# google-research/snap

Hardware: AMD Instinct MI355X
Metric: localization_scenes_per_sec (higher is better)
Workload: dtype f32 (tensors, accumulation, every non-GEMM op); conv / dense products on the bf16 matrix cores: operands split into 2 bf16 parts, 3 part products per MAC, ~2^-17 per product; 1 GPU; C2: 8 scenes/GPU, 4 StreetView views @512px + aerial, 128x128x60 voxel BEV @0.2m, ResNet-50 encoders, 10001 pose hypotheses; scenes_per_gpu=8, batches_in_flight=2, global_batch=8, parallelism=scene-sharded x1, no data-path collective, mode=inference forward (BEVLocalizer.apply, train=False)

## Files before the change

include/snap_hip.h:

```cpp
#ifndef SNAP_HIP_H_
#define SNAP_HIP_H_

#include <stddef.h>
#include <stdint.h>

#ifdef __cplusplus
extern "C" {
#endif

typedef enum SnapStatus {
  SNAP_OK = 0,
  SNAP_ERR_BAD_SHAPE = -1,
  SNAP_ERR_UNSUPPORTED = -2,
  SNAP_ERR_NULL = -3,
  SNAP_ERR_LAUNCH = -4,
  SNAP_ERR_WORKSPACE = -5
} SnapStatus;

int snap_abi_version(void);
const char* snap_status_string(int status);
const char* snap_build_arch(void);

enum { SNAP_PRO_NONE = 0, SNAP_PRO_AFFINE = 1, SNAP_PRO_GN_RELU = 2,
       SNAP_PRO_RELU_GN = 3, SNAP_PRO_RELU = 4 };
// ... 369 lines not shown

size_t snap_pose_score_workspace_bytes(int32_t B, int32_t Nq, int32_t P,
                                       int32_t X, int32_t Y);
int snap_pose_score_f32(const float* sim, const float* poses, const float* q_xy,
                        const uint8_t* valid_q, const uint8_t* map_valid,
                        int32_t B, int32_t Nq, int32_t X, int32_t Y, int32_t P,
                        float cell_size, int32_t mask_oob, float* scores,
                        void* workspace, size_t workspace_bytes, void* stream);

int snap_refine_lattice_f32(const float* init, const float* offs_r,
                            const float* offs_p, int32_t B, int32_t nr,
                            int32_t np_, float* out, void* stream);

int snap_argmax_rows_f32(const float* scores, int32_t B, int32_t P, int32_t start,
                         int32_t* idx, void* stream);

int snap_rotate_templates_f32(const float* feat, const uint8_t* valid,
                              const float* tfm, int32_t H, int32_t W, int32_t D,
                              int32_t R, float cell_size, float* templates,
                              uint8_t* tvalid, float* tw, float* cw,
                              float* tcount, void* stream);

int snap_stack_templates_f32(const float* tw, float* tws, int32_t H, int32_t W, int32_t D,
                             int32_t R, int32_t S, void* stream);
int snap_stack_templates_rhwd_f32(const float* templates, float* tws, int32_t H, int32_t W,
                                  int32_t D, int32_t R, int32_t S, void* stream);
int snap_pack_stacked_templates_split_bf16(const float* templates, int32_t H, int32_t W, int32_t D,
                                           int32_t R, int32_t S, void* out, size_t out_bytes,
                                           void* stream);
int snap_pad_map_f32(const float* map, const uint8_t* mvalid, int32_t H, int32_t W,
// ... 241 lines not shown
```

snap_amd/_lib.py:

```python
import ctypes
import os

_HERE = os.path.dirname(os.path.abspath(__file__))
LIB_PATH = os.environ.get('SNAP_HIP_LIB') or os.path.join(_HERE, 'lib', 'libsnap_hip.so')

c_int = ctypes.c_int32
c_i64 = ctypes.c_int64
c_u64 = ctypes.c_uint64
c_float = ctypes.c_float
c_size = ctypes.c_size_t
ptr = ctypes.c_void_p


class SnapConvDesc(ctypes.Structure):
  _fields_ = [
      ('N', c_int), ('H', c_int), ('W', c_int), ('Cin', c_int),
      ('Cin_stride', c_int),
      ('KH', c_int), ('KW', c_int), ('stride', c_int), ('pad_t', c_int),
      ('pad_l', c_int),
      ('Ho', c_int), ('Wo', c_int), ('Cout', c_int), ('Cout_stride', c_int),
      ('prologue', c_int), ('epilogue', c_int),
      ('in_scale', c_float), ('in_shift', c_float), ('tile_hint', c_int),
  ]

# ... 9 lines not shown
      ('bk_hint', c_int), ('tune_flags', c_int), ('gn_partial_rows', c_int), ('w_half', c_int), ('x_half', c_int), ('y_half', ptr),
      ('gnb_x', ptr), ('gnb_mu', ptr), ('gnb_rstd', ptr), ('gnb_gamma', ptr), ('gnb_beta', ptr), ('gnb_mode', c_int),
  ]


class SnapLiftDesc(ctypes.Structure):
  _fields_ = [
      ('B', c_int), ('V', c_int), ('h', c_int), ('w', c_int), ('C', c_int),
      ('feature_dim', c_int), ('num_bins', c_int), ('N', c_int), ('K', c_int),
      ('fisheye', c_int), ('out_stride', c_int),
      ('depth_min', c_float), ('depth_max', c_float),
      ('max_view_distance', c_float),
      ('weighted', c_int), ('use_variance', c_int), ('add_minmax', c_int),
      ('grid_y', c_int), ('grid_z', c_int), ('valid_rows_only', c_int), ('out_split', c_int),
      ('class_rows', c_int), ('tune_flags', c_int),
  ]


SIGNATURES = {
    'snap_abi_version': (c_int, []),
    'snap_status_string': (ctypes.c_char_p, [c_int]),
    'snap_build_arch': (ctypes.c_char_p, []),
    'snap_conv2d_nhwc_f32': (
        c_int,
        [ctypes.POINTER(SnapConvDesc), ptr, ptr, ptr, ptr, ptr, ptr, ptr, ptr,
         ptr, ptr, ptr],
    ),
    'snap_conv2d_nhwc_ex_f32': (
        c_int,
        [ctypes.POINTER(SnapConvDesc), ptr, ptr, ptr, ptr, ptr, ptr, ptr, ptr,
# ... 174 lines not shown
    'snap_poses_from_corr_f32': (
        c_int, [ptr, ptr, c_int, c_int, c_int, c_int, c_float, ptr, ptr]
    ),
    'snap_pose_score_window_workspace_bytes': (c_size, [c_int, c_int, c_int, c_int, c_int]),
    'snap_pose_score_window_supported': (c_int, [c_int, c_int, c_int]),
    'snap_pose_score_window_f32': (c_int, [ptr, ptr, ptr, c_int, ptr, ptr, c_int, c_int, c_int, c_int, c_int,
                                           c_float, ptr, ptr, c_size, ptr]),
    'snap_pose_score_workspace_bytes': (c_size, [c_int, c_int, c_int, c_int, c_int]),
    'snap_pose_score_f32': (
        c_int,
        [ptr, ptr, ptr, ptr, ptr, c_int, c_int, c_int, c_int, c_int, c_float,
         c_int, ptr, ptr, c_size, ptr],
    ),
    'snap_refine_lattice_f32': (c_int, [ptr, ptr, ptr, c_int, c_int, c_int, ptr, ptr]),
    'snap_argmax_rows_f32': (c_int, [ptr, c_int, c_int, c_int, ptr, ptr]),
    'snap_rotate_templates_f32': (
        c_int,
        [ptr, ptr, ptr, c_int, c_int, c_int, c_int, c_float, ptr, ptr, ptr, ptr,
         ptr, ptr],
    ),
    'snap_pad_map_f32': (c_int, [ptr, ptr, c_int, c_int, c_int, ptr, ptr, ptr]),
    'snap_template_finalize_f32': (
        c_int, [ptr, ptr, ptr, c_int, c_int, c_int, c_int, c_float, c_int, ptr, ptr]
    ),
    'snap_vote_peaks_workspace_bytes': (c_size, [c_int] * 6),
    'snap_vote_peaks_f32': (c_int, [ptr, c_int, c_int, c_int, c_int, c_int, c_int, ptr, ptr, ptr, ptr, c_size, ptr]),
    'snap_vote_posterior_workspace_bytes': (c_size, [c_int] * 3),
    'snap_vote_posterior_f32': (c_int, [ptr, c_int, c_int, c_int, c_float, ptr, ptr, ptr, ptr, ptr, ptr, c_size, ptr]),
    'snap_vote_fuse_workspace_bytes': (c_size, [c_int] * 4),
    'snap_vote_fuse_f32': (c_int, [ptr, ptr, ptr, c_int, c_int, c_int, c_int, ptr, ptr, ptr, c_size, ptr]),
# ... 96 lines not shown
    'snap_pose_score_bwd_f32': (
        c_int,
        [ptr, ptr, ptr, ptr, ptr, c_int, c_int, c_int, c_int, c_int, c_float, c_int, ptr, ptr,
         c_size, ptr],
    ),
    'snap_pose_score_bwd_ex_f32': (
        c_int,
        [ptr, ptr, ptr, ptr, ptr, c_int, c_int, c_int, c_int, c_int, c_float, c_int, c_int, ptr, ptr,
         c_size, ptr],
    ),
    'snap_sim_bwd_prepare_f32': (
        c_int, [ptr, ptr, c_int, c_i64, c_int, ptr, ptr, c_int, ptr]
    ),
}

ABI_VERSION = 27

_lib = None


def load():
  global _lib
  if _lib is not None:
    return _lib
  if not os.path.exists(LIB_PATH):
    raise RuntimeError(
        f'{LIB_PATH} not found: the HIP extension is not built. '
        'Run `make -C snap_amd/csrc` (needs hipcc); there is no CPU fallback.'
    )
  lib = ctypes.CDLL(LIB_PATH)
  for name, (restype, argtypes) in SIGNATURES.items():
# ... 16 lines not shown
```

snap_amd/csrc/abi.hip:

```cpp
#include "common.h"

extern "C" int snap_abi_version(void) { return 27; }

extern "C" const char* snap_build_arch(void) { return "gfx950"; }

extern "C" const char* snap_status_string(int status) {
  switch (status) {
    case SNAP_OK: return "ok";
    case SNAP_ERR_BAD_SHAPE: return "bad or inconsistent shape";
    case SNAP_ERR_UNSUPPORTED: return "unsupported option";
    case SNAP_ERR_NULL: return "required pointer is NULL";
    case SNAP_ERR_LAUNCH: return "HIP launch error";
    case SNAP_ERR_WORKSPACE: return "workspace too small";
    default: return "unknown status";
  }
}
```

snap_amd/csrc/pose.hip:

```cpp
#include <stdlib.h>

#include "common.h"
#include "philox.h"

namespace {

constexpr int SIM_CH = 64;
constexpr int SIM_TQ = 64;

template <int DM, int MODE>
__global__ __launch_bounds__(256) void sim_kernel(
    const float* __restrict__ fq, const float* __restrict__ fm, int Nq, int XY, float scale,
    int clip, const float* __restrict__ num_valid, float* __restrict__ sim,
    float* __restrict__ stats, const float* __restrict__ rowstats, float* __restrict__ prob,
    const float* __restrict__ row_weight) {
  __shared__ float q_s[SIM_TQ * DM];
  const int b = blockIdx.z;
  const int n0 = blockIdx.y * SIM_TQ;
  const int cell = blockIdx.x * 256 + threadIdx.x;
  const int lane = threadIdx.x & 63;
  const int chunk = blockIdx.x * 4 + (threadIdx.x >> 6);
  const int NC = (XY + SIM_CH - 1) / SIM_CH;
  const bool cvalid = cell < XY;
  for (int i = threadIdx.x; i < SIM_TQ * DM; i += 256) {
// ... 1305 lines not shown
  const float c = cosf(th0), s = sinf(th0);
  const float ox = offs_p[ix], oy = offs_p[iy];
  out[i * 3 + 0] = th0 + offs_r[ir];
  out[i * 3 + 1] = tx0 + (c * ox - s * oy);
  out[i * 3 + 2] = ty0 + (s * ox + c * oy);
}

__device__ __forceinline__ bool argmax_takes(float ov, int oi, float mv, int mi) {
  const bool on = ov != ov, mn = mv != mv;
  if (on != mn) return on;
  return (on || ov == mv) ? oi < mi : ov > mv;
}

template <int NT>
__global__ __launch_bounds__(NT) void argmax_rows_kernel(const float* __restrict__ scores, int P,
                                                         int start, int32_t* __restrict__ idx) {
  __shared__ float bv[NT];
  __shared__ int bi[NT];
  const int b = blockIdx.x;
  const float* row = scores + (int64_t)b * P;
  float best = -INFINITY;
  int besti = 0x7fffffff;
  for (int p = start + threadIdx.x; p < P; p += NT) {
    const float v = row[p];
    if (argmax_takes(v, p, best, besti)) { best = v; besti = p; }
  }
  bv[threadIdx.x] = best;
  bi[threadIdx.x] = besti;
  __syncthreads();
  for (int o = NT / 2; o > 0; o >>= 1) {
    if (threadIdx.x < o) {
      const float ov = bv[threadIdx.x + o];
      const int oi = bi[threadIdx.x + o];
      const float mv = bv[threadIdx.x];
      const int mi = bi[threadIdx.x];
      if (argmax_takes(ov, oi, mv, mi)) {
        bv[threadIdx.x] = ov;
        bi[threadIdx.x] = oi;
      }
    }
    __syncthreads();
  }
  if (threadIdx.x == 0) idx[b] = bi[0] - start;
}

template <int MODE>
int launch_sim(int Dm, dim3 grid, hipStream_t s, const float* fq, const float* fm, int Nq, int XY,
               float scale, int clip, const float* nv, float* sim, float* stats,
               const float* rowstats, float* prob, const float* row_weight) {
  switch (Dm) {
    case 8: hipLaunchKernelGGL((sim_kernel<8, MODE>), grid, dim3(256), 0, s, fq, fm, Nq, XY, scale, clip, nv, sim, stats, rowstats, prob, row_weight); break;
    case 16: hipLaunchKernelGGL((sim_kernel<16, MODE>), grid, dim3(256), 0, s, fq, fm, Nq, XY, scale, clip, nv, sim, stats, rowstats, prob, row_weight); break;
    case 32: hipLaunchKernelGGL((sim_kernel<32, MODE>), grid, dim3(256), 0, s, fq, fm, Nq, XY, scale, clip, nv, sim, stats, rowstats, prob, row_weight); break;
    case 64: hipLaunchKernelGGL((sim_kernel<64, MODE>), grid, dim3(256), 0, s, fq, fm, Nq, XY, scale, clip, nv, sim, stats, rowstats, prob, row_weight); break;
    default: return SNAP_ERR_UNSUPPORTED;
  }
  SNAP_CHECK_LAUNCH();
  return SNAP_OK;
// ... 334 lines not shown
  if (!init || !offs_r || !offs_p || !out) return SNAP_ERR_NULL;
  if (B <= 0 || nr <= 0 || np_ <= 0) return SNAP_ERR_BAD_SHAPE;
  const int64_t total = (int64_t)B * nr * np_ * np_;
  hipLaunchKernelGGL(refine_lattice_kernel, dim3((unsigned)snap_cdiv(total, 256)), dim3(256), 0,
                     static_cast<hipStream_t>(stream), init, offs_r, offs_p, B, nr, np_, out);
  SNAP_CHECK_LAUNCH();
  return SNAP_OK;
}

extern "C" int snap_argmax_rows_f32(const float* scores, int32_t B, int32_t P, int32_t start,
                                    int32_t* idx, void* stream) {
  if (!scores || !idx) return SNAP_ERR_NULL;
  if (B <= 0 || P <= 0 || start < 0 || start >= P) return SNAP_ERR_BAD_SHAPE;
  if (P - start > 4096)
    hipLaunchKernelGGL(argmax_rows_kernel<1024>, dim3(B), dim3(1024), 0, static_cast<hipStream_t>(stream),
                       scores, P, start, idx);
  else
    hipLaunchKernelGGL(argmax_rows_kernel<256>, dim3(B), dim3(256), 0, static_cast<hipStream_t>(stream),
                       scores, P, start, idx);
  SNAP_CHECK_LAUNCH();
  return SNAP_OK;
}
```

snap_amd/models/bev_localizer.py:

```python
import math

import numpy as np
import torch

from snap_amd import autograd as ag
from snap_amd import ops
from snap_amd.configs import defaults as default_configs
from snap_amd.models import base
from snap_amd.models import bev_mapper
from snap_amd.models import pose_estimation
from snap_amd.models import types
from snap_amd.utils import geometry
from snap_amd.utils import grids


def build_query_frustum_grid(cell_size, depth, filter_points_in_fov=False, hfov_deg=None):
  width = 3 * depth // 2
  grid = grids.Grid2D.from_extent_meters((width, depth), cell_size)
  grid_p_view = torch.tensor([width / 2, 0.0], dtype=torch.float32)
  qgrid_xy_p = grid.index_to_xyz(grid.grid_index().to(torch.float32))
  q_xy_p = qgrid_xy_p - grid_p_view
  if filter_points_in_fov:
    angle = torch.atan2(q_xy_p[..., 0], q_xy_p[..., 1])
    keep = torch.abs(angle) < math.radians(hfov_deg / 2)
# ... 83 lines not shown
        features=[f[: B * V].reshape(B, V, *f.shape[1:]) for f in pyr.features],
        strides=pyr.strides,
    )
    data_query['image_feature_pyr'] = types.FeatureImagePyramid(
        features=[f[B * V:].reshape(B, Vq, *f.shape[1:]) for f in pyr.features],
        strides=pyr.strides,
    )

  def _prefetch_scale(self, params):
    if self.config.add_temperature:
      ops.prefetch_exp(params.get('temperature'))

  def similarity(self, params, f_p_q, plane_map, valid_points, want_prob=False, conf_p=None):
    cfg = self.config
    temperature = params['temperature'] if cfg.add_temperature else None
    num_valid = valid_points.sum(-1).clamp(min=1).to(torch.float32)
    fq, fm = f_p_q.contiguous(), plane_map.features.contiguous()
    clip = bool(cfg.clip_negative_scores)
    weights = row_cdf = None
    train_w = conf_p is not None and base.needs_grad(fq, fm, temperature, conf_p)
    if conf_p is not None:
      if train_w:
        weights, row_cdf = ag.masked_softmax_rows(conf_p, valid_points)
      else:
        weights, row_cdf = ops.masked_softmax_rows(conf_p.contiguous(), valid_points.contiguous())
    if train_w:
      sim, stats, prob, scale = ag.sim_softmax_weighted(fq, fm, temperature, weights, clip, num_valid,
                                                        want_prob)
      weights, row_cdf = weights.detach(), row_cdf.detach()
    elif base.needs_grad(fq, fm, temperature):
      sim, stats, prob, scale = ag.sim_softmax(fq, fm, temperature, clip, num_valid, want_prob)
    else:
      scale = 1.0 if temperature is None else ops.host_exp(temperature)
      sim, stats, prob, _ = ops.sim_softmax(fq, fm, scale, clip, num_valid, want_prob=want_prob,
                                            row_weight=weights)
    if weights is not None:
      row_unscale = torch.where(weights > 0, 1.0 / weights.clamp(min=1e-38), torch.zeros_like(weights))
    else:
      row_unscale = num_valid[:, None].expand(-1, fq.shape[1]).contiguous()
    matching = dict(fq=fq.detach(), fm=fm.detach(), chunk_stats=stats, scale=scale, clip=clip,
                    row_cdf=row_cdf, sim=sim.detach(), row_unscale=row_unscale.contiguous())
    return sim, prob, matching

  def __call__(self, params, data, train=False, debug=False, rng=None,
               pose_samples=None):
    cfg = self.config
    ctx = base.ForwardContext()
    dev = data['query']['images'].device
    batch_size = len(data['query']['images'])
    q_xy_p = base.device_const('q_xy_p', dev, lambda: self.q_xy_p, owner=self)[None].expand(
        batch_size, -1, -1, -1)

    pred = {}
    data_map, data_query = dict(data['map']), {**data['query'], 'xy_bev': q_xy_p}
    self._prefetch_scale(params)
    self.bev_mapper.start_aerial(params['bev_mapper'], data_map, train, ctx)
    try:
      self._encode_views_jointly(params, data_map, data_query, train, ctx)
      pred['map'] = self.bev_mapper(params['bev_mapper'], data_map, train, debug, ctx=ctx, rng=rng)
    finally:
      pending = data_map.pop('_aerial_async', None)
      if pending is not None:
        torch.cuda.current_stream().wait_event(pending[1])
    mapper_q = self.bev_mapper_query or self.bev_mapper
    params_q = params['bev_mapper_query'] if self.bev_mapper_query is not None else params['bev_mapper']
    pred['query'] = mapper_q(
        params_q, data_query, train, debug, is_query=True, ctx=ctx, rng=rng,
    )

    plane_map = pred['map']['bev_matching']
    plane_q = pred['query']['bev_matching']
    q_xy_p = q_xy_p.squeeze(2).contiguous()
    valid_points = plane_q.valid.reshape(batch_size, -1)
    f_p_q = plane_q.features.reshape(batch_size, -1, plane_q.features.shape[-1])

    conf_p = None
    if cfg.add_confidence_query:
      conf_p = pred['query']['bev_confidence'].reshape(batch_size, -1)
    sim_points, prob_points, matching = self.similarity(
        params, f_p_q, plane_map, valid_points, want_prob=debug, conf_p=conf_p
    )
    if debug:
      pred['sim_points'] = sim_points
      pred['prob_points'] = prob_points

    if pose_samples is None:
      if cfg.num_pose_samples is None:
        raise ValueError('config.num_pose_samples must be set')
      m_t_q, corr = pose_estimation.sample_transforms_ransac_batched(
          rng, matching, q_xy_p, cfg.num_pose_samples,
          cfg.num_pose_sampling_retries, self.grid_map,
      )
      if debug:
        pred['correspondences'] = corr
    else:
      m_t_q = pose_samples
    m_t_q_gt = data.get('T_query2map')
    if m_t_q_gt is not None:
      m_t_q_gt = geometry.Transform2D.from_Transform3D(m_t_q_gt)
      m_t_q = geometry.Transform2D.cat([m_t_q_gt[:, None], m_t_q], 1)
    pred['map_t_query_samples'] = m_t_q

    pred['scores_poses'] = scores = pose_estimation.pose_scoring_many_batched(
        m_t_q, sim_points, q_xy_p, valid_points, plane_map.valid, self.grid_map,
        cfg.mask_score_out_of_bounds,
    )
    start_idx = int(m_t_q_gt is not None)
    pred['best_index'] = best_idx = ops.argmax_rows(scores, start_idx)
    bi = torch.arange(batch_size, device=dev)
    pred['map_t_query'] = m_t_q[bi, best_idx.to(torch.int64) + start_idx]

    if cfg.do_grid_refinement:
      pred['map_t_query_ransac'] = pred['map_t_query']
      pred['map_t_query'], pred['scores_grid_refine'] = (
          pose_estimation.grid_refinement_batched(
              pred['map_t_query'], sim_points, q_xy_p, valid_points,
              plane_map.valid, self.grid_map, cfg.mask_score_out_of_bounds,
              max_point_norm=float(self.q_xy_p.norm(dim=-1).max()),
          )
      )
    return pred

  default_config = staticmethod(default_configs.bev_localizer)


# ... 48 lines not shown
```

snap_amd/models/bev_mapper.py:

```python
import torch

from snap_amd import autograd as ag
from snap_amd import ops
from snap_amd.configs import defaults as default_configs
from snap_amd.models import base
from snap_amd.models import image_encoder
from snap_amd.models import layers
from snap_amd.models import semantic_raster_encoder
from snap_amd.models import streetview_encoder
from snap_amd.models import types


class VerticalPooling(base.Module):

  def __init__(self, config, dtype=torch.float32, num_levels=None, feature_dim=None):
    if config.pooling not in ('max', 'sum', 'mean', 'softmax', 'weighted', 'mlp'):
      raise NotImplementedError(config.pooling)
    self.config = config
    self.feature_dim = feature_dim
    self.fusion_mlp = None
    if config.pooling == 'mlp':
      if num_levels is None or feature_dim is None:
        raise ValueError("pooling='mlp' needs num_levels and feature_dim")
      self.fusion_mlp = layers.MLP(config.mlp, in_dim=num_levels * feature_dim)
# ... 101 lines not shown
          'kernel': base.truncated_normal(gen, (self.feature_dim, dm), std, device),
          'bias': torch.zeros(dm, device=device),
      }
    if self.config.add_confidence:
      params['confidence_head'] = {'layers_0': {
          'kernel': base.lecun_normal(gen, (self.feature_dim, 1), self.feature_dim, device),
          'bias': torch.zeros(1, device=device),
      }}
    return params

  def build_xyz_query(self, data, train, is_query, rng=None):
    cfg = self.config
    scene_t_view = data['T_view2scene']
    t = scene_t_view.t
    xy = data.get('xy_bev')
    if xy is None:
      xy = self.grid.index_to_xyz(self.grid.grid_index(device=t.device).to(t.dtype))
    if xy.dim() != 4:
      xy = xy[None].expand(len(t), *xy.shape)
    z_offset = data.get('z_offset')
    if z_offset is None:
      camera_heights = _median_lower_upper_mean(t[..., -1])
      z_offset = camera_heights - cfg.get('scene_z_offset', 4.0)
      if train and is_query and cfg.get('scene_z_offset_range') is not None:
        z_min, z_max = cfg.get('scene_z_offset_range')
        gen = torch.Generator(device='cpu')
        gen.manual_seed(0 if rng is None else int(rng) + 7919)
        u = torch.rand(z_offset.shape, generator=gen)
        if z_offset.is_cuda and z_offset.dtype == torch.float32:
          u = ops.upload_table(u.numpy(), z_offset.device).view(torch.float32).reshape(z_offset.shape)
        else:
          u = u.to(z_offset)
        z_offset = z_offset + (z_min + (z_max - z_min) * u)
    scene_z_height = cfg.get('scene_z_height', 12.0)
    cell = self.grid.cell_size
    nz = len(torch.arange(0, scene_z_height, cell))
    z = (
        torch.arange(nz, device=t.device, dtype=t.dtype)[None] * cell
        + z_offset[:, None]
        + cell / 2
    )
    B, X, Y = xy.shape[:3]
    if t.is_cuda and t.dtype == torch.float32 and ops.NATIVE_GLUE and not base.needs_grad(z, xy):
      xy_c = xy[0].contiguous() if xy.stride(0) == 0 else xy.contiguous()
      return ops.voxel_points(xy_c, z.contiguous())
    xyz = torch.empty(B, X, Y, nz, 3, dtype=t.dtype, device=t.device)
    xyz[..., :2] = xy[:, :, :, None, :]
    xyz[..., 2] = z[:, None, None, :]
    return xyz

  def encode_streetview(self, params, data, train, is_query, ctx=None, rng=None):
    if 'xyz_query' not in data:
      data['xyz_query'] = self.build_xyz_query(data, train, is_query, rng)
    pool_max = (not self.config.get('materialize_volume', True)
                and self.vertical_pooling.config.pooling == 'max')
    pred = self.streetview_encoder(params['streetview_encoder'], data, train=train, ctx=ctx,
                                   pool_max=pool_max)
# ... 124 lines not shown
```

snap_amd/models/pose_estimation.py:

```python
import numpy as np
import torch

from snap_amd import autograd as ag
from snap_amd import ops
from snap_amd.utils import geometry


def pose_scoring_many_batched(
    j_t_i, scores_points_all, i_xy_points, valid_points, valid_j, grid,
    mask_out_of_bounds,
):
  score = ag.pose_score if (torch.is_grad_enabled() and scores_points_all.requires_grad) else ops.pose_score
  return score(
      scores_points_all, j_t_i.packed().detach(), i_xy_points.contiguous(),
      valid_points.contiguous(), valid_j.contiguous(), grid.cell_size,
      mask_oob=mask_out_of_bounds,
  )


def sample_transforms_ransac_batched(
    rng, matching, i_xy_p, num_poses, num_retries, grid, uniforms=None,
):
  S = num_poses * num_retries * 2
  corr = ops.ransac_sample(
# ... 40 lines not shown
    range_p = float(np.abs(np.mgrid[slice(-4, 4 + 0.2, 0.2)]).max())
    range_r = float(np.deg2rad(np.abs(np.mgrid[slice(-5, 5 + 0.25, 0.25)]).max()))
    radius = int(np.ceil((range_p * np.sqrt(2.0) + float(max_point_norm) * range_r) / grid.cell_size * 1.0001)) + 1
    if not ops.pose_score_window_supported(X, Y, radius):
      radius = None
  if radius is not None:
    scores = ops.pose_score_window(
        scores_points_all, samples, init.contiguous(), radius, i_xy_points.contiguous(),
        valid_points.contiguous(), grid.cell_size)
  else:
    scores = ops.pose_score(
        scores_points_all, samples, i_xy_points.contiguous(),
        valid_points.contiguous(), valid_j.contiguous(), grid.cell_size,
        mask_oob=mask_out_of_bounds,
    )
  best = ops.argmax_rows(scores).to(torch.int64)
  B = samples.shape[0]
  refined = samples[torch.arange(B, device=dev), best]
  nr, np_ = offs_r.numel(), offs_p.numel()
  return geometry.Transform2D.from_packed(refined), scores.reshape(B, nr, np_, np_)
```

snap_amd/models/streetview_encoder.py:

```python
import copy

import numpy as np
import torch

from snap_amd import autograd as ag
from snap_amd import ops
from snap_amd.configs import defaults as default_configs
from snap_amd.models import base
from snap_amd.models import image_encoder
from snap_amd.models import layers
from snap_amd.models import types


class StreetViewEncoder(base.Module):

  def __init__(self, config, dtype=torch.float32):
    if config.pretrained_path is not None:
      raise NotImplementedError(
          'pretrained_path: Flax checkpoint loading is out of scope '
          '(and broken in the reference, streetview_encoder.py:189).'
      )
    self.config = config
    self.image_encoder = image_encoder.ImageEncoder(config.image_encoder, dtype)
    fd = config.feature_dim
# ... 78 lines not shown
      B, V = images.shape[:2]
      pyr = self.image_encoder(
          params['image_encoder'], images.reshape(B * V, *images.shape[2:]),
          train, ctx=ctx,
      )
      f_image_pyr = types.FeatureImagePyramid(
          features=[f.reshape(B, V, *f.shape[1:]) for f in pyr.features],
          strides=pyr.strides,
      )
    f_images = f_image_pyr.features[-1]
    B, V = f_images.shape[:2]
    feature_stride = f_image_pyr.strides[-1]
    inv_stride = tuple(float(v) for v in (1.0 / feature_stride[::-1]))
    scale = base.device_const(('camera_scale', inv_stride), f_images.device,
                              lambda: torch.tensor(inv_stride, dtype=torch.float32))
    cameras = data['camera'].scale(scale)
    scene_t_view = data['T_view2scene']
    pred = {'image_feature_pyramid': f_image_pyr}

    if self.weighted:
      f_images = self._project(params['proj_mlp'], f_images, train)
      pred['scores_images'] = f_images[..., -cfg.num_scale_bins:]
    else:
      f_images = f_images.contiguous()

    xyz = data['xyz_query']
    xyz_flat = xyz.reshape(len(xyz), -1, 3).contiguous()
    k_vs = cfg.top_k_view_selection
    K = k_vs if (k_vs and V > k_vs) else 0
    kw = dict(K=K, fisheye=cameras.is_fisheye, feature_dim=cfg.feature_dim,
              num_bins=cfg.num_scale_bins, depth_min_max=cfg.depth_min_max,
              max_view_distance=cfg.get('max_view_distance'))
# ... 15 lines not shown
      split = (fused and ops.POOLED_SPLIT and not cfg.fusion.apply_input_activation
               and cfg.feature_dim % 8 == 0 and (K or V) <= 4 and f_images.numel() * 4 < 2 ** 32)
      if fused:
        kw.update(valid_rows_only=True, out_split=split)
        classed = split and ops.CLASS_ROWS and cfg.feature_dim % 16 == 0
        kw.update(class_rows=classed)
        records = classed and ops.LIFT_IN_CONSUMER
        kw.update(tap_records=records)
      if not self.default_fusion:
        kw.update(weighted=self.weighted, use_variance=bool(cfg.fusion_use_variance),
                  add_minmax=bool(cfg.fusion_add_minmax))
    cam_p = rt_p = None
    if self.depth_mlp is not None:
      pooled, valid = self._lift_with_depth_mlp(params, f_images, cameras, scene_t_view, xyz_flat, K, train)
    else:
      cam_p, rt_p = cameras.packed().to(torch.float32), scene_t_view.packed().to(torch.float32)
      pooled, valid, *classes = lift(f_images, cam_p, rt_p, xyz_flat, **kw)
    grid_shape = (-1, *xyz.shape[-4:-1])
    if fused:
      p = params['fusion_mlp']
      nvar = cfg.feature_dim // 16
      plane, pvalid = ops.mlp2_pool_max(
          pooled.reshape(-1, pooled.shape[-1]), (classes[0] if classed else valid).reshape(-1),
          p['Dense_0']['kernel'], p['Dense_0']['bias'], p['Dense_1']['kernel'], p['Dense_1']['bias'],
          cin=self.fusion_mlp.in_dim, Z=grid_shape[-1],
          relu_in=bool(cfg.fusion.apply_input_activation), x_split=split,
          zero_slabs=(nvar, nvar) if classed else None,
          gather=(f_images, classes[1]) if records else None)
      kw_plain = {k: v for k, v in kw.items()
                  if k not in ('valid_rows_only', 'out_split', 'class_rows', 'tap_records')}
      engine = ops.precision()
# ... 51 lines not shown
```

snap_amd/ops.py:

```python
import contextlib
import sys
import ctypes
import threading
import typing
import weakref
import os

import numpy as np
import torch

from snap_amd import _lib

PRO_NONE, PRO_AFFINE, PRO_GN_RELU, PRO_RELU_GN, PRO_RELU = 0, 1, 2, 3, 4
EPI_BIAS, EPI_RELU, EPI_RESIDUAL, EPI_UPSAMPLE2X_ADD, EPI_ROWMASK, EPI_GELU = 1, 2, 4, 8, 16, 32
POOLING = {'max': 0, 'sum': 1, 'mean': 2}
SIM_CHUNK = 64



_TUNING_DEFAULTS = {
    'OVERLAP_AERIAL': True,
    'POOLED_SPLIT': True,
    'CLASS_ROWS': True,
    'LIFT_IN_CONSUMER': True,
# ... 1596 lines not shown
  )
  _lib.check(st, 'snap_refine_lattice_f32')
  return out


def argmax_rows(scores, start=0):
  lib = _lib.load()
  _f32(scores, 'scores')
  B, P = scores.shape
  idx = torch.empty((B,), dtype=torch.int32, device=scores.device)
  st = lib.snap_argmax_rows_f32(_p(scores), B, P, start, _p(idx), _stream())
  _lib.check(st, 'snap_argmax_rows_f32')
  return idx


def interpolate_nd(array, points, valid_array=None):
  lib = _lib.load()
  _f32(array, 'array'); _f32(points, 'points')
  K, n = points.shape
  if array.dim() != n + 1 or not 1 <= n <= 3:
    raise ValueError(f'interpolate_nd: array {tuple(array.shape)} vs points [K, {n}]')
  D = array.shape[-1]
  size = (ctypes.c_int32 * n)(*array.shape[:n])
  if valid_array is not None:
    _mask(valid_array, 'valid_array')
    if tuple(valid_array.shape) != tuple(array.shape[:n]):
      raise ValueError('interpolate_nd: valid_array shape')
  values = torch.empty((K, D), dtype=torch.float32, device=array.device)
  valid = torch.empty((K,), dtype=torch.bool, device=array.device)
  st = lib.snap_interpolate_nd_f32(_p(array), size, n, D, _p(valid_array), _p(points), K,
# ... 592 lines not shown
```

snap_amd/utils/geometry.py:

```python
import math

import torch


class _Struct:

  _fields = ()
  _event_ndim = {}

  def _map(self, fn):
    return type(self)(**{k: fn(getattr(self, k)) for k in self._fields})

  def __getitem__(self, idx):
    if not isinstance(idx, tuple):
      idx = (idx,)
    def index(k):
      v = getattr(self, k)
      nd = self._event_ndim[k]
      if any(i is Ellipsis for i in idx):
        return v[idx + (slice(None),) * nd]
      return v[idx]
    return type(self)(**{k: index(k) for k in self._fields})

  def to(self, *args, **kwargs):
# ... 66 lines not shown
      return self.transform(other)
    raise TypeError(f'Unexpected type: {type(other)}')

  def packed(self):
    return torch.cat([self.R.reshape(*self.shape, 9), self.t], -1).contiguous()


class Transform2D(_Struct):

  _fields = ('angle', 't')
  _event_ndim = {'angle': 0, 't': 1}

  def __init__(self, angle, t):
    self.angle = angle
    self.t = t

  @classmethod
  def from_radians(cls, angle, t):
    return cls(angle=angle, t=t)

  @classmethod
  def from_R(cls, R, t):
    angle = torch.atan2(R[..., 1, 0], R[..., 0, 0])
    return cls(angle, t)

  @classmethod
  def from_Transform3D(cls, transform):
    return cls.from_R(transform.R, transform.t[..., :2])

  @classmethod
  def from_packed(cls, p):
    return cls(p[..., 0], p[..., 1:])

  def packed(self):
    return torch.cat([self.angle[..., None], self.t], -1).contiguous()

  @property
  def shape(self):
    return self.angle.shape

  @property
  def R(self):
    cos, sin = torch.cos(self.angle), torch.sin(self.angle)
    return torch.stack([cos, -sin, sin, cos], -1).reshape(*self.shape, 2, 2)

  def _rotate(self, v, inverse=False, points=False):
    cos, sin = torch.cos(self.angle), torch.sin(self.angle)
    if inverse:
      sin = -sin
# ... 136 lines not shown
```

Baseline: 399.4 scenes/s.

## Replace small PyTorch glue ops with native HIP kernels across the pipeline

Adds native kernels for camera and transform packing, z-level computation with a median height, prepending the ground-truth pose, row valid-counts, and fused argmax-plus-gather. These replace chains of small PyTorch ops (cat, sum, clamp, expand, indexing) in the encoder, lifting, similarity and pose refinement. Transform2D also caches its packed tensor to avoid re-concatenating. The goal is fewer kernel launches and less host overhead per scene, at the cost of extra code paths with strict dtype and shape guards.

Result: no change. 400.2 scenes/s (median of 6 runs) (+0.2%).

```diff
diff --git a/include/snap_hip.h b/include/snap_hip.h
--- a/include/snap_hip.h
+++ b/include/snap_hip.h
@@ -407,6 +407,30 @@
 
 int snap_argmax_rows_f32(const float* scores, int32_t B, int32_t P, int32_t start,
                          int32_t* idx, void* stream);
+int snap_argmax_gather_f32(const float* scores, int32_t B, int32_t P, int32_t start, const float* rows,
+                           int32_t* idx, float* sel, void* stream);
+int snap_row_counts_f32(const uint8_t* valid, int32_t B, int32_t N, float* num_valid, float* row_unscale,
+                        void* stream);
+
+typedef struct SnapStrided {
+  const float* p;
+  int64_t sb, sv, se, se2;
+} SnapStrided;
+
+typedef struct SnapGlueViews {
+  int32_t B, V;
+  SnapStrided R, t;
+  SnapStrided wh, f, c;
+  SnapStrided k_radial, max_fov;
+  float scale_x, scale_y;
+} SnapGlueViews;
+
+int snap_glue_pack_views_f32(const SnapGlueViews* g, float* cam, float* Rt, void* stream);
+int snap_glue_z_levels_f32(const SnapStrided* t, int32_t B, int32_t V, const float* z_offset,
+                           int64_t z_offset_stride, float scene_z_offset, float cell, float half_cell,
+                           int32_t nz, float* z, void* stream);
+int snap_glue_prepend_pose_f32(const SnapStrided* R, const SnapStrided* t, const SnapStrided* angle,
+                               const SnapStrided* pt, int32_t B, int32_t P, float* out, void* stream);
 
 int snap_rotate_templates_f32(const float* feat, const uint8_t* valid,
                               const float* tfm, int32_t H, int32_t W, int32_t D,
diff --git a/snap_amd/_lib.py b/snap_amd/_lib.py
--- a/snap_amd/_lib.py
+++ b/snap_amd/_lib.py
@@ -47,6 +47,19 @@
       ('weighted', c_int), ('use_variance', c_int), ('add_minmax', c_int),
       ('grid_y', c_int), ('grid_z', c_int), ('valid_rows_only', c_int), ('out_split', c_int),
       ('class_rows', c_int), ('tune_flags', c_int),
+  ]
+
+
+class SnapStrided(ctypes.Structure):
+  _fields_ = [('p', ptr), ('sb', c_i64), ('sv', c_i64), ('se', c_i64), ('se2', c_i64)]
+
+
+class SnapGlueViews(ctypes.Structure):
+  _fields_ = [
+      ('B', c_int), ('V', c_int),
+      ('R', SnapStrided), ('t', SnapStrided), ('wh', SnapStrided), ('f', SnapStrided), ('c', SnapStrided),
+      ('k_radial', SnapStrided), ('max_fov', SnapStrided),
+      ('scale_x', c_float), ('scale_y', c_float),
   ]
 
 
@@ -251,6 +264,14 @@
     ),
     'snap_refine_lattice_f32': (c_int, [ptr, ptr, ptr, c_int, c_int, c_int, ptr, ptr]),
     'snap_argmax_rows_f32': (c_int, [ptr, c_int, c_int, c_int, ptr, ptr]),
+    'snap_argmax_gather_f32': (c_int, [ptr, c_int, c_int, c_int, ptr, ptr, ptr, ptr]),
+    'snap_row_counts_f32': (c_int, [ptr, c_int, c_int, ptr, ptr, ptr]),
+    'snap_glue_pack_views_f32': (c_int, [ctypes.POINTER(SnapGlueViews), ptr, ptr, ptr]),
+    'snap_glue_z_levels_f32': (c_int, [ctypes.POINTER(SnapStrided), c_int, c_int, ptr, c_i64, c_float, c_float,
+                                       c_float, c_int, ptr, ptr]),
+    'snap_glue_prepend_pose_f32': (c_int, [ctypes.POINTER(SnapStrided), ctypes.POINTER(SnapStrided),
+                                           ctypes.POINTER(SnapStrided), ctypes.POINTER(SnapStrided), c_int, c_int,
+                                           ptr, ptr]),
     'snap_rotate_templates_f32': (
         c_int,
         [ptr, ptr, ptr, c_int, c_int, c_int, c_int, c_float, ptr, ptr, ptr, ptr,
@@ -377,7 +398,7 @@
     ),
 }
 
-ABI_VERSION = 27
+ABI_VERSION = 28
 
 _lib = None
 
diff --git a/snap_amd/csrc/abi.hip b/snap_amd/csrc/abi.hip
--- a/snap_amd/csrc/abi.hip
+++ b/snap_amd/csrc/abi.hip
@@ -1,6 +1,6 @@
 #include "common.h"
 
-extern "C" int snap_abi_version(void) { return 27; }
+extern "C" int snap_abi_version(void) { return 28; }
 
 extern "C" const char* snap_build_arch(void) { return "gfx950"; }
 
diff --git a/snap_amd/csrc/glue_pack.h b/snap_amd/csrc/glue_pack.h
--- /dev/null
+++ b/snap_amd/csrc/glue_pack.h
@@ -0,0 +1,89 @@
+#ifndef SNAP_CSRC_GLUE_PACK_H_
+#define SNAP_CSRC_GLUE_PACK_H_
+
+#include <math.h>
+#include <stdint.h>
+
+#include "snap_hip.h"
+
+#if defined(__HIPCC__)
+#define SNAP_HD __host__ __device__ inline
+#else
+#define SNAP_HD inline
+#endif
+
+#define SNAP_GLUE_PI_F 3.14159265358979323846f
+
+SNAP_HD const float* glue_at(const SnapStrided& a, int64_t b, int64_t v) { return a.p + b * a.sb + v * a.sv; }
+
+SNAP_HD void glue_pack_camera(const SnapGlueViews& g, int64_t b, int64_t v, float* out) {
+  const float* wh = glue_at(g.wh, b, v);
+  const float* f = glue_at(g.f, b, v);
+  const float* c = glue_at(g.c, b, v);
+  out[0] = wh[0] * g.scale_x;
+  out[1] = wh[g.wh.se] * g.scale_y;
+  out[2] = f[0] * g.scale_x;
+  out[3] = f[g.f.se] * g.scale_y;
+  out[4] = c[0] * g.scale_x;
+  out[5] = c[g.c.se] * g.scale_y;
+  if (g.k_radial.p) {
+    const float* k = glue_at(g.k_radial, b, v);
+    const float fov = *glue_at(g.max_fov, b, v);
+    out[6] = k[0];
+    out[7] = k[g.k_radial.se];
+    out[8] = k[2 * g.k_radial.se];
+    out[9] = fov;
+    out[10] = tanf(0.5f * fov);
+  } else {
+    out[6] = out[7] = out[8] = 0.f;
+    out[9] = SNAP_GLUE_PI_F;
+    out[10] = 0.f;
+  }
+}
+
+SNAP_HD void glue_pack_transform(const SnapGlueViews& g, int64_t b, int64_t v, float* out) {
+  const float* R = glue_at(g.R, b, v);
+  const float* t = glue_at(g.t, b, v);
+  for (int i = 0; i < 3; ++i)
+    for (int j = 0; j < 3; ++j) out[i * 3 + j] = R[i * g.R.se + j * g.R.se2];
+  for (int i = 0; i < 3; ++i) out[9 + i] = t[i * g.t.se];
+}
+
+SNAP_HD bool glue_sorts_before(float a, int64_t ia, float b, int64_t ib) {
+  const bool an = a != a, bn = b != b;
+  if (an != bn) return bn;
+  if (an || a == b) return ia < ib;
+  return a < b;
+}
+
+SNAP_HD float glue_height_at_rank(const SnapStrided& t, int64_t b, int V, int rank) {
+  for (int i = 0; i < V; ++i) {
+    const float vi = glue_at(t, b, i)[2 * t.se];
+    int r = 0;
+    for (int j = 0; j < V; ++j) r += glue_sorts_before(glue_at(t, b, j)[2 * t.se], j, vi, i) ? 1 : 0;
+    if (r == rank) return vi;
+  }
+  return 0.f;
+}
+
+SNAP_HD float glue_z_offset(const SnapStrided& t, const float* z_offset, int64_t z_offset_stride, int64_t b, int V,
+                            float scene_z_offset) {
+  if (z_offset) return z_offset[b * z_offset_stride];
+  const float lo = glue_height_at_rank(t, b, V, (V - 1) / 2), hi = glue_height_at_rank(t, b, V, V / 2);
+  const float median = 0.5f * (lo + hi);
+  return median - scene_z_offset;
+}
+
+SNAP_HD float glue_z_level(int k, float cell, float z_offset, float half_cell) {
+  return ((float)k * cell + z_offset) + half_cell;
+}
+
+SNAP_HD void glue_pose_from_transform(const SnapStrided& R, const SnapStrided& t, int64_t b, float* out) {
+  const float* Rb = R.p + b * R.sb;
+  const float* tb = t.p + b * t.sb;
+  out[0] = atan2f(Rb[R.se], Rb[0]);
+  out[1] = tb[0];
+  out[2] = tb[t.se];
+}
+
+#endif
diff --git a/snap_amd/csrc/glue_pack.hip b/snap_amd/csrc/glue_pack.hip
--- /dev/null
+++ b/snap_amd/csrc/glue_pack.hip
@@ -0,0 +1,76 @@
+#include "common.h"
+#include "glue_pack.h"
+
+namespace {
+
+__global__ __launch_bounds__(64) void glue_pack_views_kernel(SnapGlueViews g, float* __restrict__ cam,
+                                                             float* __restrict__ Rt) {
+  const int i = blockIdx.x * 64 + threadIdx.x;
+  if (i >= g.B * g.V) return;
+  const int b = i / g.V, v = i % g.V;
+  glue_pack_camera(g, b, v, cam + (int64_t)i * 11);
+  glue_pack_transform(g, b, v, Rt + (int64_t)i * 12);
+}
+
+__global__ __launch_bounds__(64) void glue_z_levels_kernel(SnapStrided t, int V, const float* __restrict__ z_offset,
+                                                           int64_t z_offset_stride, float scene_z_offset, float cell,
+                                                           float half_cell, int nz, float* __restrict__ z) {
+  const int b = blockIdx.x;
+  const float off = glue_z_offset(t, z_offset, z_offset_stride, b, V, scene_z_offset);
+  for (int k = threadIdx.x; k < nz; k += 64) z[(int64_t)b * nz + k] = glue_z_level(k, cell, off, half_cell);
+}
+
+__global__ __launch_bounds__(256) void glue_prepend_pose_kernel(SnapStrided R, SnapStrided t, SnapStrided angle,
+                                                                SnapStrided pt, int B, int P,
+                                                                float* __restrict__ out) {
+  const int64_t i = (int64_t)blockIdx.x * 256 + threadIdx.x;
+  if (i >= (int64_t)B * (P + 1)) return;
+  const int64_t b = i / (P + 1), p = i % (P + 1);
+  float* o = out + i * 3;
+  if (p == 0) {
+    glue_pose_from_transform(R, t, b, o);
+    return;
+  }
+  const float* tp = glue_at(pt, b, p - 1);
+  o[0] = *glue_at(angle, b, p - 1);
+  o[1] = tp[0];
+  o[2] = tp[pt.se];
+}
+
+}
+
+extern "C" int snap_glue_pack_views_f32(const SnapGlueViews* g, float* cam, float* Rt, void* stream) {
+  if (!g || !cam || !Rt || !g->R.p || !g->t.p || !g->wh.p || !g->f.p || !g->c.p) return SNAP_ERR_NULL;
+  if (g->k_radial.p && !g->max_fov.p) return SNAP_ERR_NULL;
+  if (g->B <= 0 || g->V <= 0 || (int64_t)g->B * g->V > (1 << 24)) return SNAP_ERR_BAD_SHAPE;
+  const int n = g->B * g->V;
+  hipLaunchKernelGGL(glue_pack_views_kernel, dim3((unsigned)snap_cdiv(n, 64)), dim3(64), 0,
+                     static_cast<hipStream_t>(stream), *g, cam, Rt);
+  SNAP_CHECK_LAUNCH();
+  return SNAP_OK;
+}
+
+extern "C" int snap_glue_z_levels_f32(const SnapStrided* t, int32_t B, int32_t V, const float* z_offset,
+                                      int64_t z_offset_stride, float scene_z_offset, float cell, float half_cell,
+                                      int32_t nz, float* z, void* stream) {
+  if (!z || (!z_offset && (!t || !t->p))) return SNAP_ERR_NULL;
+  if (B <= 0 || nz <= 0 || (!z_offset && V <= 0)) return SNAP_ERR_BAD_SHAPE;
+  SnapStrided tt = {nullptr, 0, 0, 0, 0};
+  if (t) tt = *t;
+  hipLaunchKernelGGL(glue_z_levels_kernel, dim3(B), dim3(64), 0, static_cast<hipStream_t>(stream), tt, V, z_offset,
+                     z_offset_stride, scene_z_offset, cell, half_cell, nz, z);
+  SNAP_CHECK_LAUNCH();
+  return SNAP_OK;
+}
+
+extern "C" int snap_glue_prepend_pose_f32(const SnapStrided* R, const SnapStrided* t, const SnapStrided* angle,
+                                          const SnapStrided* pt, int32_t B, int32_t P, float* out, void* stream) {
+  if (!R || !t || !angle || !pt || !R->p || !t->p || !out) return SNAP_ERR_NULL;
+  if (B <= 0 || P < 0) return SNAP_ERR_BAD_SHAPE;
+  if (P > 0 && (!angle->p || !pt->p)) return SNAP_ERR_NULL;
+  const int64_t total = (int64_t)B * (P + 1);
+  hipLaunchKernelGGL(glue_prepend_pose_kernel, dim3((unsigned)snap_cdiv(total, 256)), dim3(256), 0,
+                     static_cast<hipStream_t>(stream), *R, *t, *angle, *pt, B, P, out);
+  SNAP_CHECK_LAUNCH();
+  return SNAP_OK;
+}
diff --git a/snap_amd/csrc/pose.hip b/snap_amd/csrc/pose.hip
--- a/snap_amd/csrc/pose.hip
+++ b/snap_amd/csrc/pose.hip
@@ -1343,7 +1343,8 @@
 
 template <int NT>
 __global__ __launch_bounds__(NT) void argmax_rows_kernel(const float* __restrict__ scores, int P,
-                                                         int start, int32_t* __restrict__ idx) {
+                                                         int start, int32_t* __restrict__ idx,
+                                                         const float* __restrict__ rows, float* __restrict__ sel) {
   __shared__ float bv[NT];
   __shared__ int bi[NT];
   const int b = blockIdx.x;
@@ -1371,6 +1372,27 @@
     __syncthreads();
   }
   if (threadIdx.x == 0) idx[b] = bi[0] - start;
+  if (rows && threadIdx.x < 3) sel[b * 3 + threadIdx.x] = rows[((int64_t)b * P + bi[0]) * 3 + threadIdx.x];
+}
+
+__global__ __launch_bounds__(256) void row_counts_kernel(const uint8_t* __restrict__ valid, int N,
+                                                         float* __restrict__ num_valid,
+                                                         float* __restrict__ row_unscale) {
+  __shared__ int cnt[256];
+  const int b = blockIdx.x;
+  const uint8_t* row = valid + (int64_t)b * N;
+  int c = 0;
+  for (int n = threadIdx.x; n < N; n += 256) c += row[n] != 0;
+  cnt[threadIdx.x] = c;
+  __syncthreads();
+  for (int o = 128; o > 0; o >>= 1) {
+    if (threadIdx.x < o) cnt[threadIdx.x] += cnt[threadIdx.x + o];
+    __syncthreads();
+  }
+  const float nv = (float)(cnt[0] < 1 ? 1 : cnt[0]);
+  if (threadIdx.x == 0) num_valid[b] = nv;
+  if (row_unscale)
+    for (int n = threadIdx.x; n < N; n += 256) row_unscale[(int64_t)b * N + n] = nv;
 }
 
 template <int MODE>
@@ -1735,10 +1757,34 @@
   if (B <= 0 || P <= 0 || start < 0 || start >= P) return SNAP_ERR_BAD_SHAPE;
   if (P - start > 4096)
     hipLaunchKernelGGL(argmax_rows_kernel<1024>, dim3(B), dim3(1024), 0, static_cast<hipStream_t>(stream),
-                       scores, P, start, idx);
+                       scores, P, start, idx, (const float*)nullptr, (float*)nullptr);
   else
     hipLaunchKernelGGL(argmax_rows_kernel<256>, dim3(B), dim3(256), 0, static_cast<hipStream_t>(stream),
-                       scores, P, start, idx);
+                       scores, P, start, idx, (const float*)nullptr, (float*)nullptr);
   SNAP_CHECK_LAUNCH();
   return SNAP_OK;
 }
+
+extern "C" int snap_argmax_gather_f32(const float* scores, int32_t B, int32_t P, int32_t start, const float* rows,
+                                      int32_t* idx, float* sel, void* stream) {
+  if (!scores || !idx || !rows || !sel) return SNAP_ERR_NULL;
+  if (B <= 0 || P <= 0 || start < 0 || start >= P) return SNAP_ERR_BAD_SHAPE;
+  if (P - start > 4096)
+    hipLaunchKernelGGL(argmax_rows_kernel<1024>, dim3(B), dim3(1024), 0, static_cast<hipStream_t>(stream),
+                       scores, P, start, idx, rows, sel);
+  else
+    hipLaunchKernelGGL(argmax_rows_kernel<256>, dim3(B), dim3(256), 0, static_cast<hipStream_t>(stream),
+                       scores, P, start, idx, rows, sel);
+  SNAP_CHECK_LAUNCH();
+  return SNAP_OK;
+}
+
+extern "C" int snap_row_counts_f32(const uint8_t* valid, int32_t B, int32_t N, float* num_valid, float* row_unscale,
+                                   void* stream) {
+  if (!valid || !num_valid) return SNAP_ERR_NULL;
+  if (B <= 0 || N <= 0) return SNAP_ERR_BAD_SHAPE;
+  hipLaunchKernelGGL(row_counts_kernel, dim3(B), dim3(256), 0, static_cast<hipStream_t>(stream), valid, N,
+                     num_valid, row_unscale);
+  SNAP_CHECK_LAUNCH();
+  return SNAP_OK;
+}
diff --git a/snap_amd/models/bev_localizer.py b/snap_amd/models/bev_localizer.py
--- a/snap_amd/models/bev_localizer.py
+++ b/snap_amd/models/bev_localizer.py
@@ -121,7 +121,11 @@
   def similarity(self, params, f_p_q, plane_map, valid_points, want_prob=False, conf_p=None):
     cfg = self.config
     temperature = params['temperature'] if cfg.add_temperature else None
-    num_valid = valid_points.sum(-1).clamp(min=1).to(torch.float32)
+    rows_nv = None
+    if valid_points.is_cuda and ops.NATIVE_GLUE and valid_points.dtype == torch.bool:
+      num_valid, rows_nv = ops.row_counts(valid_points.contiguous(), want_rows=conf_p is None)
+    else:
+      num_valid = valid_points.sum(-1).clamp(min=1).to(torch.float32)
     fq, fm = f_p_q.contiguous(), plane_map.features.contiguous()
     clip = bool(cfg.clip_negative_scores)
     weights = row_cdf = None
@@ -143,6 +147,8 @@
                                             row_weight=weights)
     if weights is not None:
       row_unscale = torch.where(weights > 0, 1.0 / weights.clamp(min=1e-38), torch.zeros_like(weights))
+    elif rows_nv is not None:
+      row_unscale = rows_nv
     else:
       row_unscale = num_valid[:, None].expand(-1, fq.shape[1]).contiguous()
     matching = dict(fq=fq.detach(), fm=fm.detach(), chunk_stats=stats, scale=scale, clip=clip,
@@ -157,6 +163,7 @@
     batch_size = len(data['query']['images'])
     q_xy_p = base.device_const('q_xy_p', dev, lambda: self.q_xy_p, owner=self)[None].expand(
         batch_size, -1, -1, -1)
+    native = dev.type == 'cuda' and ops.NATIVE_GLUE and not train
 
     pred = {}
     data_map, data_query = dict(data['map']), {**data['query'], 'xy_bev': q_xy_p}
@@ -177,7 +184,11 @@
 
     plane_map = pred['map']['bev_matching']
     plane_q = pred['query']['bev_matching']
-    q_xy_p = q_xy_p.squeeze(2).contiguous()
+    if native:
+      q_xy_p = base.device_const(('q_xy_p_batch', batch_size), dev,
+                                 lambda: self.q_xy_p.squeeze(1)[None].repeat(batch_size, 1, 1), owner=self)
+    else:
+      q_xy_p = q_xy_p.squeeze(2).contiguous()
     valid_points = plane_q.valid.reshape(batch_size, -1)
     f_p_q = plane_q.features.reshape(batch_size, -1, plane_q.features.shape[-1])
 
@@ -204,8 +215,13 @@
       m_t_q = pose_samples
     m_t_q_gt = data.get('T_query2map')
     if m_t_q_gt is not None:
-      m_t_q_gt = geometry.Transform2D.from_Transform3D(m_t_q_gt)
-      m_t_q = geometry.Transform2D.cat([m_t_q_gt[:, None], m_t_q], 1)
+      if (native and m_t_q.angle.dim() == 2 and m_t_q_gt.t.dim() == 2
+          and all(t.dtype == torch.float32 for t in (m_t_q_gt.R, m_t_q_gt.t, m_t_q.angle, m_t_q.t))
+          and not base.needs_grad(m_t_q_gt.R, m_t_q_gt.t, m_t_q.angle, m_t_q.t)):
+        m_t_q = geometry.Transform2D.from_packed(ops.glue_prepend_pose(m_t_q_gt, m_t_q))
+      else:
+        m_t_q_gt = geometry.Transform2D.from_Transform3D(m_t_q_gt)
+        m_t_q = geometry.Transform2D.cat([m_t_q_gt[:, None], m_t_q], 1)
     pred['map_t_query_samples'] = m_t_q
 
     pred['scores_poses'] = scores = pose_estimation.pose_scoring_many_batched(
@@ -213,9 +229,13 @@
         cfg.mask_score_out_of_bounds,
     )
     start_idx = int(m_t_q_gt is not None)
-    pred['best_index'] = best_idx = ops.argmax_rows(scores, start_idx)
-    bi = torch.arange(batch_size, device=dev)
-    pred['map_t_query'] = m_t_q[bi, best_idx.to(torch.int64) + start_idx]
+    if native and scores.dtype == torch.float32 and not base.needs_grad(m_t_q.angle, m_t_q.t):
+      pred['best_index'], best = ops.argmax_gather(scores.detach(), m_t_q.packed(), start_idx)
+      pred['map_t_query'] = geometry.Transform2D.from_packed(best)
+    else:
+      pred['best_index'] = best_idx = ops.argmax_rows(scores, start_idx)
+      bi = torch.arange(batch_size, device=dev)
+      pred['map_t_query'] = m_t_q[bi, best_idx.to(torch.int64) + start_idx]
 
     if cfg.do_grid_refinement:
       pred['map_t_query_ransac'] = pred['map_t_query']
diff --git a/snap_amd/models/bev_mapper.py b/snap_amd/models/bev_mapper.py
--- a/snap_amd/models/bev_mapper.py
+++ b/snap_amd/models/bev_mapper.py
@@ -139,15 +139,31 @@
     scene_t_view = data['T_view2scene']
     t = scene_t_view.t
     xy = data.get('xy_bev')
+    native = t.is_cuda and t.dtype == torch.float32 and ops.NATIVE_GLUE and t.dim() == 3 and not base.needs_grad(t)
     if xy is None:
-      xy = self.grid.index_to_xyz(self.grid.grid_index(device=t.device).to(t.dtype))
+      if native:
+        xy = base.device_const('grid_xy', t.device,
+                               lambda: self.grid.index_to_xyz(self.grid.grid_index().to(t.dtype)), owner=self)
+      else:
+        xy = self.grid.index_to_xyz(self.grid.grid_index(device=t.device).to(t.dtype))
     if xy.dim() != 4:
       xy = xy[None].expand(len(t), *xy.shape)
     z_offset = data.get('z_offset')
+    scene_z_height = cfg.get('scene_z_height', 12.0)
+    cell = self.grid.cell_size
+    nz = len(torch.arange(0, scene_z_height, cell))
+    B, X, Y = xy.shape[:3]
+    jitter = train and is_query and cfg.get('scene_z_offset_range') is not None
+    if (native and not jitter and not base.needs_grad(xy) and xy.is_cuda and xy.dtype == torch.float32
+        and (z_offset is None or (z_offset.is_cuda and z_offset.dtype == torch.float32
+                                  and tuple(z_offset.shape) == (B,) and not base.needs_grad(z_offset)))):
+      z = ops.glue_z_levels(t, nz, cell, cfg.get('scene_z_offset', 4.0), z_offset)
+      xy_c = xy[0].contiguous() if xy.stride(0) == 0 else xy.contiguous()
+      return ops.voxel_points(xy_c, z)
     if z_offset is None:
       camera_heights = _median_lower_upper_mean(t[..., -1])
       z_offset = camera_heights - cfg.get('scene_z_offset', 4.0)
-      if train and is_query and cfg.get('scene_z_offset_range') is not None:
+      if jitter:
         z_min, z_max = cfg.get('scene_z_offset_range')
         gen = torch.Generator(device='cpu')
         gen.manual_seed(0 if rng is None else int(rng) + 7919)
@@ -157,15 +173,11 @@
         else:
           u = u.to(z_offset)
         z_offset = z_offset + (z_min + (z_max - z_min) * u)
-    scene_z_height = cfg.get('scene_z_height', 12.0)
-    cell = self.grid.cell_size
-    nz = len(torch.arange(0, scene_z_height, cell))
     z = (
         torch.arange(nz, device=t.device, dtype=t.dtype)[None] * cell
         + z_offset[:, None]
         + cell / 2
     )
-    B, X, Y = xy.shape[:3]
     if t.is_cuda and t.dtype == torch.float32 and ops.NATIVE_GLUE and not base.needs_grad(z, xy):
       xy_c = xy[0].contiguous() if xy.stride(0) == 0 else xy.contiguous()
       return ops.voxel_points(xy_c, z.contiguous())
diff --git a/snap_amd/models/pose_estimation.py b/snap_amd/models/pose_estimation.py
--- a/snap_amd/models/pose_estimation.py
+++ b/snap_amd/models/pose_estimation.py
@@ -78,8 +78,11 @@
         valid_points.contiguous(), valid_j.contiguous(), grid.cell_size,
         mask_oob=mask_out_of_bounds,
     )
-  best = ops.argmax_rows(scores).to(torch.int64)
   B = samples.shape[0]
-  refined = samples[torch.arange(B, device=dev), best]
+  if ops.NATIVE_GLUE and scores.is_cuda:
+    _, refined = ops.argmax_gather(scores, samples)
+  else:
+    best = ops.argmax_rows(scores).to(torch.int64)
+    refined = samples[torch.arange(B, device=dev), best]
   nr, np_ = offs_r.numel(), offs_p.numel()
   return geometry.Transform2D.from_packed(refined), scores.reshape(B, nr, np_, np_)
diff --git a/snap_amd/models/streetview_encoder.py b/snap_amd/models/streetview_encoder.py
--- a/snap_amd/models/streetview_encoder.py
+++ b/snap_amd/models/streetview_encoder.py
@@ -116,8 +116,16 @@
     inv_stride = tuple(float(v) for v in (1.0 / feature_stride[::-1]))
     scale = base.device_const(('camera_scale', inv_stride), f_images.device,
                               lambda: torch.tensor(inv_stride, dtype=torch.float32))
-    cameras = data['camera'].scale(scale)
     scene_t_view = data['T_view2scene']
+    packed = None
+    cam0 = data['camera']
+    fields = [cam0.wh, cam0.f, cam0.c, scene_t_view.R, scene_t_view.t]
+    if cam0.is_fisheye:
+      fields += [cam0.k_radial, cam0.max_fov]
+    if (not train and ops.NATIVE_GLUE and self.depth_mlp is None and scene_t_view.t.dim() == 3
+        and all(t.is_cuda and t.dtype == torch.float32 for t in fields) and not base.needs_grad(*fields)):
+      packed = ops.glue_pack_views(cam0, scene_t_view, inv_stride)
+    cameras = cam0.scale(scale) if packed is None else cam0
     pred = {'image_feature_pyramid': f_image_pyr}
 
     if self.weighted:
@@ -163,7 +171,7 @@
     if self.depth_mlp is not None:
       pooled, valid = self._lift_with_depth_mlp(params, f_images, cameras, scene_t_view, xyz_flat, K, train)
     else:
-      cam_p, rt_p = cameras.packed().to(torch.float32), scene_t_view.packed().to(torch.float32)
+      cam_p, rt_p = packed or (cameras.packed().to(torch.float32), scene_t_view.packed().to(torch.float32))
       pooled, valid, *classes = lift(f_images, cam_p, rt_p, xyz_flat, **kw)
     grid_shape = (-1, *xyz.shape[-4:-1])
     if fused:
diff --git a/snap_amd/ops.py b/snap_amd/ops.py
--- a/snap_amd/ops.py
+++ b/snap_amd/ops.py
@@ -1634,6 +1634,95 @@
   return idx
 
 
+def argmax_gather(scores, rows, start=0):
+  lib = _lib.load()
+  _f32(scores, 'scores'); _f32(rows, 'rows')
+  B, P = scores.shape
+  if tuple(rows.shape) != (B, P, 3):
+    raise ValueError('argmax_gather: rows must be [B, P, 3]')
+  idx = torch.empty((B,), dtype=torch.int32, device=scores.device)
+  sel = torch.empty((B, 3), dtype=torch.float32, device=scores.device)
+  st = lib.snap_argmax_gather_f32(_p(scores), B, P, start, _p(rows), _p(idx), _p(sel), _stream())
+  _lib.check(st, 'snap_argmax_gather_f32')
+  return idx, sel
+
+
+def row_counts(valid, want_rows=True):
+  lib = _lib.load()
+  _mask(valid, 'valid')
+  B, N = valid.shape
+  num_valid = torch.empty((B,), dtype=torch.float32, device=valid.device)
+  rows = torch.empty((B, N), dtype=torch.float32, device=valid.device) if want_rows else None
+  st = lib.snap_row_counts_f32(_p(valid), B, N, _p(num_valid), _p(rows), _stream())
+  _lib.check(st, 'snap_row_counts_f32')
+  return num_valid, rows
+
+
+def _strided(t, lead, name):
+  if t is None:
+    return _lib.SnapStrided(None, 0, 0, 0, 0)
+  if not isinstance(t, torch.Tensor) or not t.is_cuda or t.dtype != torch.float32:
+    raise TypeError(f'{name}: expected a float32 tensor on a ROCm GPU (any strides)')
+  st = list(t.stride())
+  sb = st[0]
+  sv = st[1] if lead == 2 else 0
+  ev = st[lead:] + [0, 0]
+  return _lib.SnapStrided(t.data_ptr(), sb, sv, ev[0], ev[1])
+
+
+def _chk_views(t, shape, name):
+  if tuple(t.shape) != tuple(shape):
+    raise ValueError(f'{name}: expected {tuple(shape)}, got {tuple(t.shape)}')
+  return t
+
+
+def glue_pack_views(camera, transform, scale_xy):
+  lib = _lib.load()
+  B, V = transform.t.shape[:2]
+  fisheye = bool(camera.is_fisheye)
+  g = _lib.SnapGlueViews(
+      B, V,
+      _strided(_chk_views(transform.R, (B, V, 3, 3), 'R'), 2, 'R'), _strided(_chk_views(transform.t, (B, V, 3), 't'), 2, 't'),
+      _strided(_chk_views(camera.wh, (B, V, 2), 'wh'), 2, 'wh'), _strided(_chk_views(camera.f, (B, V, 2), 'f'), 2, 'f'),
+      _strided(_chk_views(camera.c, (B, V, 2), 'c'), 2, 'c'),
+      _strided(_chk_views(camera.k_radial, (B, V, 3), 'k_radial') if fisheye else None, 2, 'k_radial'),
+      _strided(_chk_views(camera.max_fov, (B, V), 'max_fov') if fisheye else None, 2, 'max_fov'),
+      float(scale_xy[0]), float(scale_xy[1]))
+  dev = transform.t.device
+  cam = torch.empty((B, V, 11), dtype=torch.float32, device=dev)
+  Rt = torch.empty((B, V, 12), dtype=torch.float32, device=dev)
+  st = lib.snap_glue_pack_views_f32(ctypes.byref(g), _p(cam), _p(Rt), _stream())
+  _lib.check(st, 'snap_glue_pack_views_f32')
+  return cam, Rt
+
+
+def glue_z_levels(t, nz, cell, scene_z_offset, z_offset=None):
+  lib = _lib.load()
+  B, V = t.shape[:2]
+  ts = _strided(_chk_views(t, (B, V, 3), 't'), 2, 't')
+  if z_offset is not None:
+    _strided(_chk_views(z_offset, (B,), 'z_offset'), 1, 'z_offset')
+  z = torch.empty((B, int(nz)), dtype=torch.float32, device=t.device)
+  st = lib.snap_glue_z_levels_f32(
+      ctypes.byref(ts), B, V, _p(z_offset), 0 if z_offset is None else z_offset.stride(0), float(scene_z_offset),
+      float(cell), float(cell / 2), int(nz), _p(z), _stream())
+  _lib.check(st, 'snap_glue_z_levels_f32')
+  return z
+
+
+def glue_prepend_pose(T_gt, poses):
+  lib = _lib.load()
+  B, P = poses.angle.shape
+  _chk_views(T_gt.R, (B, 3, 3), 'R'); _chk_views(T_gt.t, (B, 3), 't'); _chk_views(poses.t, (B, P, 2), 'poses.t')
+  R, t = _strided(T_gt.R, 1, 'R'), _strided(T_gt.t, 1, 't')
+  a, pt = _strided(poses.angle, 2, 'angle'), _strided(poses.t, 2, 'poses.t')
+  out = torch.empty((B, P + 1, 3), dtype=torch.float32, device=poses.angle.device)
+  st = lib.snap_glue_prepend_pose_f32(ctypes.byref(R), ctypes.byref(t), ctypes.byref(a), ctypes.byref(pt), B, P,
+                                      _p(out), _stream())
+  _lib.check(st, 'snap_glue_prepend_pose_f32')
+  return out
+
+
 def interpolate_nd(array, points, valid_array=None):
   lib = _lib.load()
   _f32(array, 'array'); _f32(points, 'points')
diff --git a/snap_amd/utils/geometry.py b/snap_amd/utils/geometry.py
--- a/snap_amd/utils/geometry.py
+++ b/snap_amd/utils/geometry.py
@@ -104,6 +104,7 @@
   def __init__(self, angle, t):
     self.angle = angle
     self.t = t
+    self._packed = None
 
   @classmethod
   def from_radians(cls, angle, t):
@@ -120,9 +121,14 @@
 
   @classmethod
   def from_packed(cls, p):
-    return cls(p[..., 0], p[..., 1:])
-
-  def packed(self):
+    out = cls(p[..., 0], p[..., 1:])
+    if p.is_contiguous():
+      out._packed = p
+    return out
+
+  def packed(self):
+    if self._packed is not None:
+      return self._packed
     return torch.cat([self.angle[..., None], self.t], -1).contiguous()
 
   @property
```
